# theoneinaminion/FVENS

Measured on AMD Instinct MI355X. Metric: Mfaces/s (flux+residual sweep) + achieved HBM GB/s, 1/2/4/8 MI355X, higher is better.
Workload: dtype f64; 1 GPU; cells=4063232, faces=6359040, boundary_faces=4096, ntheta=2048, nquad=256, ntri=864, farmap=1, parallelism=single GPU

## Files before the change

fvens_amd/csrc/ctx.hpp:

```cpp
#ifndef FVHIP_CTX_HPP
#define FVHIP_CTX_HPP

#include "../../include/fvhip.h"
#include "layout.hpp"
#include "kernels.hpp"
#include "jacobian.hpp"
#include "mesh.hpp"
#include "partition.hpp"
#include "halo.hpp"
#include "ode.hpp"
#include "surface.hpp"
#include "amg.hpp"
#include <rccl/rccl.h>
#include <hip/hip_runtime.h>
#include <cstring>
#include <cstdio>
#include <cstdlib>
#include <algorithm>
#include <cmath>
#include <string>
#include <vector>
#include <map>
#include <stdexcept>
#include <memory>
// ... 91 lines not shown
		double *z = nullptr, *aux = nullptr;
		double *w = nullptr, *t = nullptr, *s = nullptr, *du = nullptr, *yg = nullptr;
		double *jd = nullptr, *jlo = nullptr, *jup = nullptr, *dinv = nullptr;
		float *slo = nullptr, *sup = nullptr, *sdinv = nullptr;
		float* sdiag = nullptr;
		double *part = nullptr, *red = nullptr, *coef = nullptr, *pm = nullptr;
		double *h_red = nullptr, *h_coef = nullptr, *h_red2 = nullptr;
	} iw;
	std::vector<void*> owned_host;
	JacMesh J{};
	bool jac_ready = false;
	double *d_jb = nullptr, *d_jlo = nullptr, *d_jup = nullptr, *d_jdiag = nullptr;
	double* d_raw = nullptr;
	size_t raw_cap = 0;
	double* rawScratch(size_t doubles) {
		if(raw_cap < doubles) {
			if(d_raw) { HC(hipStreamSynchronize(stream)); release(d_raw); }
			d_raw = dalloc(doubles, owned);
			raw_cap = doubles;
		}
		return d_raw;
	}
	int rank = 0, nparts = 1;
	bool rankmesh = false;
	bool use_staged = false;
	bool use_pipe = false;
	int* d_pipe_patch = nullptr;
	hipStream_t stream2 = nullptr;
	std::vector<hipEvent_t> pipe_ev;
	hipEvent_t pipe_start = nullptr, pipe_done = nullptr;
	ncclComm_t comm = nullptr;
	bool in_group = false;
	int* d_fz_order = nullptr;
	hipStream_t comm_stream = nullptr;
	hipEvent_t ev_u = nullptr, ev_halo = nullptr;
	hipEvent_t ev_packed = nullptr, ev_copied = nullptr;
	bool copied_recorded = false;
	int* d_send = nullptr;
	int* d_border = nullptr;
	int nborder = 0;
	double* d_sendbuf = nullptr;
	int* d_trace_conn = nullptr;
	double* d_tracebuf = nullptr;
	int nsend = 0;
	bool prof = false;
	struct Rec { std::string name; hipEvent_t a, b; };
	std::vector<Rec> recs;
	std::map<std::string, std::pair<double,int>> acc;

	~fvhip_ctx() {
		(void)hipSetDevice(device);
		if(comm) (void)ncclCommDestroy(comm);
		for(auto& r : recs) { (void)hipEventDestroy(r.a); (void)hipEventDestroy(r.b); }
		for(hipEvent_t e : pipe_ev) (void)hipEventDestroy(e);
		if(pipe_start) (void)hipEventDestroy(pipe_start);
		if(pipe_done) (void)hipEventDestroy(pipe_done);
		if(stream2) (void)hipStreamDestroy(stream2);
		if(ev_u) (void)hipEventDestroy(ev_u);
		if(ev_halo) (void)hipEventDestroy(ev_halo);
		if(ev_packed) (void)hipEventDestroy(ev_packed);
		if(ev_copied) (void)hipEventDestroy(ev_copied);
		if(comm_stream) (void)hipStreamDestroy(comm_stream);
		for(void* p : owned) (void)hipFree(p);
		for(void* p : owned_host) (void)hipHostFree(p);
		if(stream) (void)hipStreamDestroy(stream);
	}
// ... 89 lines not shown
			HC(hipStreamCreateWithFlags(&stream2, hipStreamNonBlocking));
			pipe_ev.resize(K);
			for(hipEvent_t& e : pipe_ev) HC(hipEventCreateWithFlags(&e, hipEventDisableTiming));
			HC(hipEventCreateWithFlags(&pipe_start, hipEventDisableTiming));
			HC(hipEventCreateWithFlags(&pipe_done, hipEventDisableTiming));
		}
		HC(hipEventRecord(pipe_start, stream));
		HC(hipStreamWaitEvent(stream2, pipe_start, 0));
		for(int k = 0; k < K; k++) {
			timed("k_prep_grad_wls", [&]{
				KOPS(launch_prep_grad_wls)(M, P, u, d_up, d_ubc, d_ug, d_grad, stream, L.pipe_cell_start[k], L.pipe_cell_start[k+1], 0, nullptr);
			});
			HC(hipEventRecord(pipe_ev[k], stream));
		}
		for(int k = 0; k < K; k++) {
			const int n = L.pipe_group_start[k+1] - L.pipe_group_start[k];
			if(n == 0) continue;
			HC(hipStreamWaitEvent(stream2, pipe_ev[k], 0));
			stage_sweep(u, r, dt, dtm, overwrite, d_pipe_patch + L.pipe_group_start[k], n, stream2);
		}
		HC(hipEventRecord(pipe_done, stream2));
		HC(hipStreamWaitEvent(stream, pipe_done, 0));
	}
	void stage_fused(const double* u, double* r, bool dt, double* dtm, bool overwrite,
	                 const int* plist = nullptr, int pcount = 0, hipStream_t st = nullptr) {
		if(!st) st = stream;
		SweepBuffers B{};
		B.u = u; B.r = r; B.dtm = dtm; B.overwrite = overwrite ? 1 : 0;
		B.plist = plist; B.pcount = pcount;
		if(plist && pcount == 0) return;
		B.grad = d_grad;
		if(limited()) B.phi = d_phi;
		B.mfx = mfz.x; B.mfpm = mfz.pm; B.mfres = mfz.res; B.mfmdt = mfz.mdt;
		const char* nm = nullptr;
		timed_on(st, "k_residual_wls", [&]{ nm = KOPS(launch_residual_wls)(M, P, B, cfg.conv_numflux, recKind(), viscKind(),
		                                                                       limKind(), dt, st); });
		if(prof && !recs.empty() && recs.back().name == "k_residual_wls" && nm) recs.back().name = nm;
		HC(hipGetLastError());
	}

	struct MfFuse { const double *x = nullptr, *pm = nullptr, *res = nullptr, *mdt = nullptr; } mfz;
	bool matfreeFusable() const { return fused() && !halo(); }
	bool matfreeNoAlias(const double* u, const double* x, const double* y) const {
		const size_t n = 4*static_cast<size_t>(L.ncell), nt = 4*static_cast<size_t>(L.ncell + L.nghost);
		auto apart = [](const double* a, size_t na, const double* b, size_t nb) { return a + na <= b || b + nb <= a; };
		return apart(y, n, x, nt) && apart(y, n, u, nt);
	}
	void matfree_fused(const double* u, const double* x, const double* pm, const double* res, const double* mdt, double* y) {
		if(!matfreeFusable()) throw std::logic_error("matfree_fused: not a fused single-domain configuration");
		mfz = MfFuse{x, pm, res, mdt};
		try { stage_fused(u, y, false, nullptr, true); }
		catch(...) { mfz = MfFuse{}; throw; }
		mfz = MfFuse{};
	}

	void pack(const double* arr, int width, hipStream_t st = nullptr) {
		if(!st) st = stream;
		timed_on(st, "k_pack", [&]{ launch_pack_rows(d_send, nsend, arr, width, d_sendbuf, st); });
	}
	int sendCount(size_t k, int layers) const {
		return (layers >= 2 || L.send_l1_end.empty() ? L.send_start[k+1] : L.send_l1_end[k]) - L.send_start[k];
	}
	int ghostCount(size_t k, int layers) const {
		return (layers >= 2 || L.ghost_l1_end.empty() ? L.ghost_start[k+1] : L.ghost_l1_end[k]) - L.ghost_start[k];
	}
	void trace_pack(const double* left, int width, hipStream_t st) {
// ... 376 lines not shown
```

fvens_amd/csrc/fvhip_api.cpp:

```cpp
#include "ctx.hpp"

#include <cmath>

namespace fvhip_detail {

fvhip_ctx::GroupExchange groupExchange(const fvhip_group_s* g)
{
	return [g](const fvhip_ctx::ArrayOf& arr_of, int width, int layers) {
		const std::vector<fvhip_ctx*>& hs = g->hs;
		const size_t n = hs.size();
		std::vector<fvhip_ctx*> byrank(n);
		for(fvhip_ctx* h : hs) byrank[h->rank] = h;
		for(size_t i = 0; i < n; i++) if(hs[i]->halo()) { HC(hipSetDevice(hs[i]->device)); hs[i]->pack(arr_of(i), width); }
		for(size_t i = 0; i < n; i++) HC(hipStreamSynchronize(hs[i]->stream));
		for(size_t i = 0; i < n; i++) {
			fvhip_ctx* h = hs[i];
			const Layout& L = h->L;
			for(size_t k = 0; k < L.nbr_rank.size(); k++) {
				fvhip_ctx* q = byrank[L.nbr_rank[k]];
				const Layout& Q = q->L;
				size_t kk = 0;
				while(kk < Q.nbr_rank.size() && Q.nbr_rank[kk] != h->rank) kk++;
				if(kk == Q.nbr_rank.size()) throw std::logic_error("halo lists are not symmetric");
				const int cnt = h->ghostCount(k, layers);
// ... 57 lines not shown
	DevMesh& M = h->M;
	M.ncell = L.ncell + L.nghost; M.nown = L.ncell; M.nbface = L.nbface;
	M.npatch = static_cast<int>(L.patch_cell.size()) - 1;
	M.nslot = static_cast<int>(L.slot_L.size());
	M.patch_cell = upload(L.patch_cell, o);
	M.patch_slot = upload(L.patch_slot, o);
	M.slot_LR = reinterpret_cast<const int2*>(upload(pack2(L.slot_L, L.slot_R), o));
	M.slot_n = reinterpret_cast<const double2*>(upload(L.slot_n, o));
	M.slot_len = upload(L.slot_len, o);
	M.slot_gr = reinterpret_cast<const double2*>(upload(L.slot_gr, o));
	M.cell_slots = reinterpret_cast<const int4*>(upload(L.cell_slots, o));
	M.cell_nbr = reinterpret_cast<const int4*>(upload(L.cell_nbr_local, o));
	M.cell_face = reinterpret_cast<const int4*>(upload(L.cell_face_local, o));
	M.cell_nbr_fo = reinterpret_cast<const int4*>(upload(L.cell_nbr_fo, o));
	M.rc = reinterpret_cast<const double2*>(upload(L.rc, o));
	M.area = upload(L.area, o);
	M.wls_V = reinterpret_cast<const double4*>(upload(L.wls_V, o));
	M.venk_eps2 = upload(L.venk_eps2, o);
	M.bf_L = upload(L.bf_L, o);
	M.bf_bc = upload(L.bf_bc, o);
	M.bf_n = reinterpret_cast<const double2*>(upload(L.bf_n, o));
	M.bf_rcbp = reinterpret_cast<const double2*>(upload(L.bf_rcbp, o));
	if(!L.fz_ext_start.empty()) {
		M.fz_ext_start = upload(L.fz_ext_start, o);
		M.fz_ext = upload(L.fz_ext, o);
		M.fz_n1 = upload(L.fz_n1, o);
		M.fz_g_start = upload(L.fz_g_start, o);
		M.fz_gnbr = reinterpret_cast<const int4*>(upload(L.fz_gnbr, o));
		M.fz_slot_lr16 = upload(L.fz_slot_lr16, o);
		M.fz_gnbr16 = reinterpret_cast<const uint2*>(upload(L.fz_gnbr16, o));
		M.fz_gbf_start = upload(L.fz_gbf_start, o);
		M.fz_gbf = upload(L.fz_gbf, o);
		M.fz_cslot16 = reinterpret_cast<const uint2*>(upload(L.fz_cslot16, o));
		M.fz_max_cells = L.fz_max_cells;
	}
	M.gg_n = static_cast<int>(L.gg_cells.size());
	M.gg_cells = upload(L.gg_cells, o);
	M.gg_nbr = reinterpret_cast<const int4*>(upload(L.gg_nbr, o));
	M.gg_V = reinterpret_cast<const double4*>(upload(L.gg_V, o));
	M.gg_gp = reinterpret_cast<const double2*>(upload(L.gg_gp, o));
	M.gg_eps2 = upload(L.gg_eps2, o);
	M.xb_bc = upload(L.xb_bc, o);
	M.xb_n = reinterpret_cast<const double2*>(upload(L.xb_n, o));
	M.xb_rcbp = reinterpret_cast<const double2*>(upload(L.xb_rcbp, o));
	if(!L.pipe_patch.empty()) h->d_pipe_patch = upload(L.pipe_patch, o);
	if(L.nghost > 0 && !L.fz_order.empty()) h->d_fz_order = upload(L.fz_order, o);
	h->d_perm = upload(L.perm, o);
	h->nsend = static_cast<int>(L.send_cells.size());
	h->nborder = static_cast<int>(L.border_cells.size());
	if(h->nborder > 0) h->d_border = upload(L.border_cells, o);
	if(h->nsend > 0) {
		h->d_send = upload(L.send_cells, o);
		h->d_sendbuf = dalloc(8*static_cast<size_t>(h->nsend), o);
	}
	if(!L.trace_conn.empty()) {
		if(static_cast<int>(L.trace_conn.size()) != h->nsend) throw std::logic_error("per-rank mesh: trace lists differ");
		h->d_trace_conn = upload(L.trace_conn, o);
		h->d_tracebuf = dalloc(4*static_cast<size_t>(L.nghost), o);
	}

	DevPhys& P = h->P;
	P.gas = gd::make_gas(cfg->gamma, cfg->Minf, cfg->Tinf, cfg->Reinf, cfg->Pr);
	const double beta = 0;
	P.uinf[0] = 1.0;
	P.uinf[1] = std::cos(cfg->aoa)*std::cos(beta);
	P.uinf[2] = std::sin(cfg->aoa)*std::cos(beta);
// ... 634 lines not shown
			names[static_cast<size_t>(n)*namelen + namelen-1] = '\0';
			ms[n] = kv.second.first; counts[n] = kv.second.second;
			n++;
		}
	});
	return rc ? -1 : n;
}

static void layoutStats(const Layout& L, long long* s, int n)
{
	long long v[16] = {};
	v[0] = L.ncell; v[1] = L.naface; v[2] = static_cast<long long>(L.slot_L.size());
	v[3] = static_cast<long long>(L.patch_cell.size()) - 1; v[4] = L.max_slots; v[5] = L.nbface;
	v[6] = L.nghost; v[7] = static_cast<long long>(L.nbr_rank.size()); v[8] = static_cast<long long>(L.send_cells.size());
	v[9] = L.fz_ninner;
	v[10] = static_cast<long long>(L.fz_ext.size()) - L.fz_ring2;
	const long long np = static_cast<long long>(L.patch_cell.size()) - 1;
	if(!L.fz_ext_start.empty())
		for(long long p = 0; p < np; p++) {
			const long long nl = (L.patch_cell[p+1] - L.patch_cell[p]) + (L.fz_ext_start[p+1] - L.fz_ext_start[p]);
			if(nl > SLOTS_MAX) v[11]++;
		}
	v[12] = L.fz_ring2;
	v[13] = L.fz_max_cells;
	v[14] = SLOTS_MAX;
	for(int i = 0; i < n && i < 16; i++) s[i] = v[i];
}

int fvhip_layout_stats(fvhip_handle h, long long* s)
{
	return guard([&] { need(h, "handle"); need(s, "stats"); layoutStats(h->L, s, 12); });
}

int fvhip_layout_probe(const fvhip_mesh* mesh, const fvhip_flow_config* cfg, long long* s)
{
	return guard([&] {
		if(!mesh || !cfg || !s) throw std::invalid_argument("null argument");
		checkConfig(cfg);
		const Layout L = buildLayout(topoFromMesh(*mesh), *cfg, true);
		layoutStats(L, s, 16);
	});
}

int fvhip_local_flux(int flux_type, const double* gas5, int nf, const double* ul, const double* ur,
                     const double* n, double* flux)
{
	return guard([&] {
		const gd::Gas G = gd::make_gas(gas5[0], gas5[1], gas5[2], gas5[3], gas5[4]);
		double *a, *b, *c, *d;
		HC(hipMalloc(&a, 4*sizeof(double)*nf + 8)); HC(hipMalloc(&b, 4*sizeof(double)*nf + 8));
		HC(hipMalloc(&c, 2*sizeof(double)*nf + 8)); HC(hipMalloc(&d, 4*sizeof(double)*nf + 8));
		HC(hipMemcpy(a, ul, 4*sizeof(double)*nf, hipMemcpyHostToDevice));
		HC(hipMemcpy(b, ur, 4*sizeof(double)*nf, hipMemcpyHostToDevice));
		HC(hipMemcpy(c, n, 2*sizeof(double)*nf, hipMemcpyHostToDevice));
		exact::launch_local_flux(flux_type, G, nf, a, b, c, d, nullptr);
		HC(hipGetLastError());
		HC(hipMemcpy(flux, d, 4*sizeof(double)*nf, hipMemcpyDeviceToHost));
		(void)hipFree(a); (void)hipFree(b); (void)hipFree(c); (void)hipFree(d);
	});
}

int fvhip_divsqrt_probe(int n, const double* a, const double* b, double* out)
{
	return guard([&] {
		double *da, *db, *dout;
		HC(hipMalloc(&da, sizeof(double)*n + 8)); HC(hipMalloc(&db, sizeof(double)*n + 8));
// ... 157 lines not shown
```

fvens_amd/csrc/kernels.hip:

```cpp
#include "kernels.hpp"
#include "layout.hpp"
#include <algorithm>
#include <mutex>
#include <set>
#include <stdexcept>
#include <string>

#ifndef FVHIP_NS
#define FVHIP_NS exact
#endif

namespace fvhip {
namespace FVHIP_NS {

using namespace gd;

__device__ __forceinline__ int xcd_chunk(int nchunk) {
	const int q = (nchunk + 7) >> 3;
	return (static_cast<int>(blockIdx.x) & 7) * q + (static_cast<int>(blockIdx.x) >> 3);
}
static inline int xcd_blocks(long long nchunk) { return static_cast<int>(8*((nchunk + 7)/8)); }

__device__ __forceinline__ void ld4(const double* p, int i, double* o) {
	const double4 v = reinterpret_cast<const double4*>(p)[i];
// ... 985 lines not shown
		grad[1][3] = davg[1] - ddr*dr[1] + corr*dr[1];
	}
	#pragma unroll
	for(int i = 1; i < 3; i++) {
		__asm__ volatile("" ::: "memory");
		const double tl = rowi[i], tr = rowj ? rowj[i] : (i == 1 ? gpr.y : gpr.z);
		double davg[2];
		davg[0] = 0.5*(rowi[4 + i*2 + 0] + gsrc[4 + i*2 + 0]);
		davg[1] = 0.5*(rowi[4 + i*2 + 1] + gsrc[4 + i*2 + 1]);
		const double corr = div_rn(tr-tl, dist);
		const double ddr = dot2(davg,dr);
		grad[0][i] = davg[0] - ddr*dr[0] + corr*dr[0];
		grad[1][i] = davg[1] - ddr*dr[1] + corr*dr[1];
	}
	const double kd = div_rcp(muRe, G.kden, G.rkden);
	double ldiv = 0;
	ldiv += grad[0][1]; ldiv += grad[1][2];
	ldiv *= 2.0/3.0*muRe;
	double s[2][2];
	s[0][0] = __builtin_fma(muRe*grad[0][1], 2.0, -ldiv); s[0][1] = muRe*(grad[0][2] + grad[1][1]);
	s[1][0] = muRe*(grad[1][1] + grad[0][2]); s[1][1] = __builtin_fma(muRe*grad[1][2], 2.0, -ldiv);
	vf[0] = 0;
	for(int i = 0; i < 2; i++) { double t = 0; t -= s[i][0]*n[0]; t -= s[i][1]*n[1]; vf[i+1] = t; }
	double e = 0;
	for(int i = 0; i < 2; i++) {
		double comp = 0;
		comp += s[i][0]*va[0]; comp += s[i][1]*va[1];
		comp += kd*grad[i][3];
		e -= comp * n[i];
	}
	vf[3] = e;
}

struct FzPatch { int p, s0, s1, c0, c1, nc, e0, nl, ng; const uint2* gnbr; const int* gbf; };
struct FzPre { int cf; double ua[4]; double2 rca; int4 nb4a; int2 lrl; double2 nn; double len;
               double2 gpa[4]; double eps2a; };

__device__ __forceinline__ FzPatch fz_patch(const DevMesh& M, const SweepBuffers& B, int pi)
{
	FzPatch q;
	q.p = B.plist ? B.plist[pi] : pi;
	q.s0 = M.patch_slot[q.p]; q.s1 = M.patch_slot[q.p+1];
	q.c0 = M.patch_cell[q.p]; q.c1 = M.patch_cell[q.p+1];
	q.nc = q.c1 - q.c0;
	q.e0 = M.fz_ext_start[q.p];
	q.nl = q.nc + (M.fz_ext_start[q.p+1] - q.e0);
	q.ng = q.nc + M.fz_n1[q.p];
	q.gnbr = M.fz_gnbr16 + M.fz_g_start[q.p];
	q.gbf = M.fz_gbf + M.fz_gbf_start[q.p];
	return q;
}
__device__ __forceinline__ int fz_nbr_code(unsigned x, const int* gbf)
{
	if(x == 0xFFFFu) return -1;
	if(x & 0x8000u) return -2 - gbf[x & 0x7FFFu];
	return static_cast<int>(x);
}
__device__ __forceinline__ int4 fz_nbrs(const FzPatch& q, int i)
{
	const uint2 v = q.gnbr[i];
	return make_int4(fz_nbr_code(v.x & 0xFFFFu, q.gbf), fz_nbr_code(v.x >> 16, q.gbf),
	                 fz_nbr_code(v.y & 0xFFFFu, q.gbf), fz_nbr_code(v.y >> 16, q.gbf));
}
__device__ __forceinline__ int fz_cell(const DevMesh& M, const FzPatch& q, int i)
{
	return i < q.nc ? q.c0 + i : M.fz_ext[q.e0 + (i - q.nc)];
}
template <bool MF>
__device__ __forceinline__ void fz_load_rows(const DevMesh& M, const SweepBuffers& B, const FzPatch& q, int t, FzPre& a)
{
	a.ua[0] = a.ua[1] = a.ua[2] = a.ua[3] = 0.0;
	a.rca = make_double2(0, 0);
	if(t < q.nl) { ld_state<MF>(B, a.cf, a.ua); a.rca = M.rc[a.cf]; }
	const int s = q.s0 + t;
	a.lrl = make_int2(0, -1); a.nn = make_double2(0, 0); a.len = 0;
	if(s < q.s1) {
		const unsigned v = M.fz_slot_lr16[s];
		a.lrl = make_int2(static_cast<int>(v & 0xFFFFu), (v >> 16) == 0xFFFFu ? -2 : static_cast<int>(v >> 16));
		a.nn = M.slot_n[s]; a.len = M.slot_len[s];
	}
}
__device__ __forceinline__ void fz_load_grad(const DevMesh& M, const FzPatch& q, int t, FzPre& a)
{
	a.nb4a = make_int4(-1, -1, -1, -1);
	if(t < q.ng && a.cf < M.nown) a.nb4a = fz_nbrs(q, t);
}

template <int FLUX, int REC, bool DT, int VISC, int LIM, typename HA, typename HB>
__device__ __forceinline__ void fz_body(const DevMesh& M, const DevPhys& P, const SweepBuffers& B, double* fz,
                                        const FzPatch& q, const FzPre& a, HA&& hookA, HB&& hookB)
{
	const Gas& G = P.gas;
	const int t = static_cast<int>(threadIdx.x);
	const int s = q.s0 + t;
	constexpr int W = fz_w<VISC>();

	if(t < q.nl) stage_row(G, &fz[t*W], a.ua, a.rca);
	for(int i = t + SLOTS_MAX; i < q.nl; i += SLOTS_MAX) {
		const int c = fz_cell(M, q, i);
		double b[4];
		ld_state<!DT>(B, c, b);
		stage_row(G, &fz[i*W], b, M.rc[c]);
	}
	__syncthreads();

	hookA();
	if(t < q.ng) fused_wls_row<LIM, W, !DT>(M, P, B, fz, &fz[t*W], a.cf, a.nb4a, LIM ? a.gpa : nullptr, a.eps2a);
	for(int i = t + SLOTS_MAX; i < q.ng; i += SLOTS_MAX) {
		const int c = fz_cell(M, q, i);
		fused_wls_row<LIM, W, !DT>(M, P, B, fz, &fz[i*W], c, c < M.nown ? fz_nbrs(q, i) : make_int4(-1, -1, -1, -1));
	}
	__syncthreads();

	double f[4] = {0, 0, 0, 0};
	double sri = 0, srj = 0;
	if(s < q.s1) {
		const int2 lrl = a.lrl;
		const double2 nn = a.nn;
		const double flen = a.len;
		const double n[2] = {nn.x, nn.y};
		const bool bnd = lrl.y < -1;
		int bf = 0, bcell = 0;
		if(bnd) { const int2 g = M.slot_LR[s]; bf = g.y - M.ncell; bcell = g.x; }
		double ul[4], ur[4];
		const double* rowi = &fz[lrl.x*W];
		const double2 ri = *reinterpret_cast<const double2*>(rowi + 12);
		double ui[4], gi[8];
		ld4(rowi, 0, ui);
		ld8(rowi + 4, 0, gi);
		if(REC == SR_MUSCL) {
			if(!bnd) {
				const double* rowj = &fz[lrl.y*W];
				const double2 rj = *reinterpret_cast<const double2*>(rowj + 12);
				double uj[4], gj[8];
				ld4(rowj, 0, uj);
				ld8(rowj + 4, 0, gj);
				const double dx = rj.x-ri.x, dy = rj.y-ri.y;
				#pragma unroll
				for(int i = 0; i < 4; i++) {
					double dl = mul0(gi[i*2], dx); dl += gi[i*2+1]*dy;
					double dr = mul0(gj[i*2], dx); dr += gj[i*2+1]*dy;
					const double du = uj[i] - ui[i];
					const double dm = twice_minus(dl, du);
					const double dp = twice_minus(dr, du);
					ul[i] = muscl_left(ui[i], uj[i], dm, muscl_phi(dm, du));
// ... 62 lines not shown
				if(g.x < M.nown) sri += div_rn(div_rcp(coi*mui, G.Pr, G.rPr) * flen*flen, M.area[g.x]);
				if(!bnd && g.y < M.nown) srj += div_rn(div_rcp(coj*muj, G.Pr, G.rPr) * flen*flen, M.area[g.y]);
			}
		}
		if(VISC != SV_NONE) {
			double muRe, va[2];
			viscous_face_terms_mu<VISC == SV_CONST>(G, ul, ur, mui, muj, muRe, va);
			double4 gpr = make_double4(0, 0, 0, 0);
			const double* rowj = nullptr;
			double2 rr;
			if(bnd) { gpr = ghost_prim_of_cell<!DT>(M, P, B, bcell, bf); rr = M.bf_rcbp[bf]; }
			else { rowj = &fz[lrl.y*W]; rr = *reinterpret_cast<const double2*>(rowj + 12); }
			const double4 vg = make_double4(ri.x, ri.y, rr.x, rr.y);
			double vf[4] = {0, 0, 0, 0};
			fz_viscous(G, rowi, rowj, gpr, vg, n, muRe, va, vf);
			#pragma unroll
			for(int k = 0; k < 4; k++) f[k] += vf[k]*flen;
		}
	}
	hookB();
	const int c = q.c0 + t;
	uint2 cs = make_uint2(0xFFFFFFFFu, 0xFFFFFFFFu);
	double carea = 0.0;
	if(c < q.c1) { cs = M.fz_cslot16[c]; if(DT) carea = M.area[c]; }
	__syncthreads();
	double* sf = fz;
	double* ssr = fz + 4*SLOTS_MAX;
	if(s < q.s1) {
		sf[0*SLOTS_MAX + t] = f[0]; sf[1*SLOTS_MAX + t] = f[1];
		sf[2*SLOTS_MAX + t] = f[2]; sf[3*SLOTS_MAX + t] = f[3];
		if(DT) { ssr[t] = sri; ssr[SLOTS_MAX + t] = srj; }
	}
	__syncthreads();

	if(c < q.c1) {
		double r[4];
		if(B.overwrite) { r[0] = r[1] = r[2] = r[3] = 0.0; }
		else ld4(B.r, c, r);
		double integ = 0.0;
		const unsigned e[4] = {cs.x & 0xFFFFu, cs.x >> 16, cs.y & 0xFFFFu, cs.y >> 16};
		#pragma unroll
		for(int k = 0; k < 4; k++) {
			if(e[k] == 0xFFFFu) break;
			const int ls = static_cast<int>(e[k] >> 1);
			if(e[k] & 1) {
				r[0] += sf[0*SLOTS_MAX + ls]; r[1] += sf[1*SLOTS_MAX + ls];
				r[2] += sf[2*SLOTS_MAX + ls]; r[3] += sf[3*SLOTS_MAX + ls];
				if(DT) integ += ssr[SLOTS_MAX + ls];
			} else {
				r[0] -= sf[0*SLOTS_MAX + ls]; r[1] -= sf[1*SLOTS_MAX + ls];
				r[2] -= sf[2*SLOTS_MAX + ls]; r[3] -= sf[3*SLOTS_MAX + ls];
				if(DT) integ += ssr[ls];
			}
		}
		if(!DT && B.mfx) {
			double x[4], rs[4];
			ld4(B.mfx, c, x);
			ld4(B.mfres, c, rs);
			const double d = B.mfmdt[c], pert = B.mfpm[1];
			#pragma unroll
			for(int i = 0; i < 4; i++) r[i] = d*x[i] + (-r[i] + rs[i])/pert;
		}
		st4(B.r, c, r);
		if(DT) B.dtm[c] = div_rn(carea, integ);
	}
}

#ifndef FVHIP_FUSED_WAVES
#define FVHIP_FUSED_WAVES 5
#endif
#ifndef FVHIP_FUSED_WAVES_LIM
#define FVHIP_FUSED_WAVES_LIM 4
#endif
#ifndef FVHIP_FUSED_WAVES_VISC
#define FVHIP_FUSED_WAVES_VISC 4
#endif

template <int FLUX, int REC, bool DT, int VISC, int LIM>
__global__ void __launch_bounds__(SLOTS_MAX, VISC != SV_NONE ? FVHIP_FUSED_WAVES_VISC : (LIM ? FVHIP_FUSED_WAVES_LIM : FVHIP_FUSED_WAVES)) k_residual_wls(const DevMesh M, const DevPhys P, const SweepBuffers B)
{
	extern __shared__ __attribute__((aligned(16))) double fz[];
	const int np = B.plist ? B.pcount : M.npatch;
	const int t = static_cast<int>(threadIdx.x);
	const int q = (np + 7) >> 3;
	const int pi = (blockIdx.x & 7) * q + (blockIdx.x >> 3);
	if(pi >= np) return;
	const FzPatch cur = fz_patch(M, B, pi);
	FzPre pre;
	pre.cf = t < cur.nl ? fz_cell(M, cur, t) : 0;
	fz_load_rows<!DT>(M, B, cur, t, pre);
	fz_load_grad(M, cur, t, pre);
	pre.eps2a = 0.0;
	if(LIM) {
		const bool own = t < cur.ng && pre.cf < M.nown;
		fz_face_centres(M, own ? pre.cf : 0, pre.gpa);
		if(LIM == 2) pre.eps2a = M.venk_eps2[own ? pre.cf : 0];
	}
	fz_body<FLUX, REC, DT, VISC, LIM>(M, P, B, fz, cur, pre, []() {}, []() {});
}

__global__ void k_fill(double* p, double v, long long n)
{
	const long long i = static_cast<long long>(blockIdx.x)*blockDim.x + threadIdx.x;
	if(i < n) p[i] = v;
}

__global__ void k_local_flux(int type, Gas G, int nf, const double* ul, const double* ur, const double* n, double* f)
{
	const int i = blockIdx.x*blockDim.x + threadIdx.x;
	if(i >= nf) return;
	double a[4], b[4], o[4];
	ld4(ul, i, a); ld4(ur, i, b);
	const double nn[2] = {n[2*i], n[2*i+1]};
	inviscid_flux_rt(type, G, a, b, nn, o);
	st4(f, i, o);
}

__global__ void k_gather(const int* perm, const double* src, double* dst, int n, int width)
{
	const long long i = static_cast<long long>(blockIdx.x)*blockDim.x + threadIdx.x;
	if(i >= static_cast<long long>(n)*width) return;
	const int c = static_cast<int>(i / width), w = static_cast<int>(i % width);
	dst[i] = src[static_cast<size_t>(perm[c])*width + w];
}

__global__ void k_scatter(const int* perm, const double* src, double* dst, int n, int width)
{
	const long long i = static_cast<long long>(blockIdx.x)*blockDim.x + threadIdx.x;
	if(i >= static_cast<long long>(n)*width) return;
	const int c = static_cast<int>(i / width), w = static_cast<int>(i % width);
	dst[static_cast<size_t>(perm[c])*width + w] = src[i];
// ... 150 lines not shown
const char* launch_residual_wls(const DevMesh& M, const DevPhys& P, const SweepBuffers& B, int flux, int rec,
                                int visc, int lim, bool dt, hipStream_t s)
{
	FusedFn fn;
	switch(flux) {
		case 0: fn = pickFused<0>(rec, visc, lim, dt); break;
		case 1: fn = pickFused<1>(rec, visc, lim, dt); break;
		case 2: fn = pickFused<2>(rec, visc, lim, dt); break;
		case 3: fn = pickFused<3>(rec, visc, lim, dt); break;
		case 4: fn = pickFused<4>(rec, visc, lim, dt); break;
		case 5: fn = pickFused<5>(rec, visc, lim, dt); break;
		default: fn = pickFused<6>(rec, visc, lim, dt); break;
	}
	const size_t W = visc != SV_NONE ? FZW_VISC : FZW;
	const size_t lds = std::max(static_cast<size_t>(M.fz_max_cells)*W, static_cast<size_t>(6*SLOTS_MAX))*sizeof(double);
	{
		static std::mutex mu;
		static std::set<std::pair<const void*, int>> configured;
		int dev = 0;
		if(hipGetDevice(&dev) != hipSuccess) throw std::runtime_error("k_residual_wls: hipGetDevice failed");
		std::lock_guard<std::mutex> lock(mu);
		if(configured.insert({reinterpret_cast<const void*>(fn), dev}).second) {
			const size_t maxlds = std::max(static_cast<size_t>(FUSED_LDS_CELLS)*W, static_cast<size_t>(6*SLOTS_MAX))*sizeof(double);
			const hipError_t e = hipFuncSetAttribute(reinterpret_cast<const void*>(fn),
			                                         hipFuncAttributeMaxDynamicSharedMemorySize, static_cast<int>(maxlds));
			if(e != hipSuccess) {
				configured.erase({reinterpret_cast<const void*>(fn), dev});
				throw std::runtime_error(std::string("k_residual_wls: raising the dynamic LDS limit failed: ")
				                         + hipGetErrorString(e));
			}
		}
	}
	const int np = B.plist ? B.pcount : M.npatch;
	if(np > 0) hipLaunchKernelGGL(fn, dim3(8*((np + 7)/8)), dim3(SLOTS_MAX), lds, s, M, P, B);
	return kFusedNames[flux < 0 || flux > 6 ? 6 : flux];
}

}
}
```

fvens_amd/csrc/kernels.hpp:

```cpp
#ifndef FVHIP_KERNELS_HPP
#define FVHIP_KERNELS_HPP

#include <hip/hip_runtime.h>
#include "gasdyn.hpp"

namespace fvhip {

constexpr int MAXBC = 16;

enum SweepRec { SR_FIRST = 0, SR_MUSCL = 1, SR_LINEAR = 2 };
enum SweepVisc { SV_NONE = 0, SV_SUTHERLAND = 1, SV_CONST = 2 };

struct DevMesh
{
	int ncell;
	int nown;
	int nbface, npatch, nslot;
	const int* patch_cell;
	const int* patch_slot;
	const int2* slot_LR;
	const double2* slot_n;
	const double* slot_len;
	const double2* slot_gr;
	const int4* cell_slots;
	const int4* cell_nbr;
	const int4* cell_face;
	const int4* cell_nbr_fo;
	const double2* rc;
	const double* area;
	const double4* wls_V;
	const double* venk_eps2;
	const int* bf_L;
	const int* bf_bc;
	const double2* bf_n;
	const double2* bf_rcbp;
	const int* fz_ext_start;
	const int* fz_ext;
	const int* fz_n1;
	const int* fz_g_start;
	const int4* fz_gnbr;
	const unsigned* fz_slot_lr16;
	const uint2* fz_gnbr16;
	const int* fz_gbf_start;
	const int* fz_gbf;
	const uint2* fz_cslot16;
	int fz_max_cells;
	int gg_n;
	const int* gg_cells;
	const int4* gg_nbr;
	const double4* gg_V;
	const double2* gg_gp;
	const double* gg_eps2;
	const int* xb_bc;
	const double2* xb_n;
	const double2* xb_rcbp;
};

struct DevPhys
{
	gd::Gas gas;
	double uinf[4];
	gd::BCDev bc[MAXBC];
	int nbc;
	double limiter_param;
};

struct SweepBuffers
{
	const double* u;
	const double* up;
	const double* grad;
	const double* rgrad;
	const double* phi;
	const double* ubc;
	const double* ug;
	double* r;
	double* dtm;
	int overwrite;
	const int* plist;
	int pcount;
	const double* mfx;
	const double* mfpm;
	const double* mfres;
	const double* mfmdt;
};

#define FVHIP_SWEEP_LAUNCHERS \
void launch_prep(const DevMesh& M, const DevPhys& P, const double* u, double* up, double* ubc, double* ug, \
                 bool cells, hipStream_t s); \
void launch_grad_wls(const DevMesh& M, const double* up, const double* ug, double* grad, hipStream_t s); \
void launch_prep_grad_wls(const DevMesh& M, const DevPhys& P, const double* u, double* up, double* ubc, \
                          double* ug, double* grad, hipStream_t s, int c_begin = 0, int c_end = -1, \
                          int lim = 0, double* phi = nullptr); \
void launch_grad_wls_list(const DevMesh& M, const DevPhys& P, const double* u, const int* list, int n, \
                          double* grad, hipStream_t s); \
void launch_grad_ghost(const DevMesh& M, const DevPhys& P, const double* u, double* grad, hipStream_t s, \
                       int lim = 0, double* phi = nullptr); \
void launch_grad_gg(const DevMesh& M, const double* up, const double* ug, double* grad, hipStream_t s); \
void launch_limiter(const DevMesh& M, const DevPhys& P, int venk, const double* up, const double* ug, \
                    const double* grad, double* phi, hipStream_t s); \
void launch_weno(const DevMesh& M, const DevPhys& P, const double* grad, double* lgrad, hipStream_t s); \
 \
const char* launch_sweep(const DevMesh& M, const DevPhys& P, const SweepBuffers& B, int flux, int rec, \
                         int visc, bool dt, hipStream_t s); \
const char* launch_residual_wls(const DevMesh& M, const DevPhys& P, const SweepBuffers& B, int flux, int rec, \
                                int visc, int lim, bool dt, hipStream_t s); \
void launch_fill(double* p, double v, long long n, hipStream_t s); \
void launch_local_flux(int flux, const gd::Gas& G, int nf, const double* ul, const double* ur, \
                       const double* n, double* f, hipStream_t s); \
void launch_gather_cells(const int* perm, const double* src, double* dst, int n, int width, hipStream_t s); \
void launch_scatter_cells(const int* perm, const double* src, double* dst, int n, int width, hipStream_t s); \
void launch_divsqrt_probe(int n, const double* a, const double* b, double* out, hipStream_t s);

namespace exact { FVHIP_SWEEP_LAUNCHERS }
namespace fast { FVHIP_SWEEP_LAUNCHERS }

}
// ... 2 lines not shown
```

fvens_amd/csrc/layout.cpp:

```cpp
#include <cstdlib>
#include "layout.hpp"
#include "partition.hpp"
#include <algorithm>
#include <numeric>
#include <stdexcept>
#include <string>
#include <cmath>

namespace fvhip {

namespace {

inline uint64_t hilbertD(uint32_t n, uint32_t x, uint32_t y)
{
	uint64_t d = 0;
	for(uint32_t s = n/2; s > 0; s /= 2) {
		const uint32_t rx = (x & s) > 0, ry = (y & s) > 0;
		d += static_cast<uint64_t>(s) * s * ((3 * rx) ^ ry);
		if(ry == 0) {
			if(rx == 1) { x = s-1 - x; y = s-1 - y; }
			const uint32_t t = x; x = y; y = t;
		}
	}
	return d;
// ... 493 lines not shown
			Lo.fz_slot_lr[2*static_cast<size_t>(s)] = code(Lo.slot_L[s]);
			Lo.fz_slot_lr[2*static_cast<size_t>(s)+1] = code(Lo.slot_R[s]);
		}
		const size_t gb0 = Lo.fz_gbf.size();
		for(size_t k = Lo.fz_gnbr.size() - 4*static_cast<size_t>(ng); k < Lo.fz_gnbr.size(); k++) {
			const int v = Lo.fz_gnbr[k];
			if(v == -1) { Lo.fz_gnbr16.push_back(0xFFFF); continue; }
			if(v >= 0) { Lo.fz_gnbr16.push_back(static_cast<uint16_t>(v)); continue; }
			const size_t j = Lo.fz_gbf.size() - gb0;
			if(j >= 0x7FFF) throw std::logic_error("fused residual: too many boundary faces in one patch");
			Lo.fz_gbf.push_back(-2 - v);
			Lo.fz_gnbr16.push_back(static_cast<uint16_t>(0x8000 | j));
		}
		Lo.fz_gbf_start.push_back(static_cast<int>(Lo.fz_gbf.size()));
		for(int s = Lo.patch_slot[p]; s < Lo.patch_slot[p+1]; s++) {
			const int l = Lo.fz_slot_lr[2*static_cast<size_t>(s)], r = Lo.fz_slot_lr[2*static_cast<size_t>(s)+1];
			Lo.fz_slot_lr16[s] = static_cast<uint32_t>(l) | (static_cast<uint32_t>(r >= 0 ? r : 0xFFFF) << 16);
		}
		for(int c = c0; c < c1; c++)
			for(int j = 0; j < MAXF; j++) {
				const int e = Lo.cell_slots[static_cast<size_t>(c)*MAXF+j];
				if(e < 0) continue;
				const int ls = (e >> 1) - Lo.patch_slot[p];
				if(ls < 0 || ls >= SLOTS_MAX) throw std::logic_error("fused residual: cell face outside its patch");
				Lo.fz_cslot16[static_cast<size_t>(c)*MAXF+j] = static_cast<uint16_t>((ls << 1) | (e & 1));
			}
		Lo.fz_max_cells = std::max(Lo.fz_max_cells, nl);
		bool inner = true;
		for(size_t k = e0; k < Lo.fz_ext.size(); k++) if(Lo.fz_ext[k] >= Lo.ncell) inner = false;
		innerp[p] = inner ? 1 : 0;
		for(int c = c0; c < c1; c++) lidx[c] = -1;
		for(size_t k = e0; k < Lo.fz_ext.size(); k++) lidx[Lo.fz_ext[k]] = -1;
	}
	Lo.fz_order.clear();
	for(int p = 0; p < npatch; p++) if(innerp[p]) Lo.fz_order.push_back(p);
	Lo.fz_ninner = static_cast<int>(Lo.fz_order.size());
	for(int p = 0; p < npatch; p++) if(!innerp[p]) Lo.fz_order.push_back(p);
}

}
```

fvens_amd/csrc/layout.hpp:

```cpp
#ifndef FVHIP_LAYOUT_HPP
#define FVHIP_LAYOUT_HPP

#include <vector>
#include <cstdint>
#include "../../include/fvhip.h"

namespace fvhip {

#ifndef FVHIP_SLOTS
#define FVHIP_SLOTS 256
#endif
#ifndef FVHIP_FUSED_ROWS
#define FVHIP_FUSED_ROWS (FVHIP_SLOTS*11/8)
#endif
constexpr int SLOTS_MAX = FVHIP_SLOTS;
constexpr int CELLS_MAX = FVHIP_SLOTS;
constexpr int MAXF = 4;

struct Layout
{
	int ncell = 0;
	int nghost = 0;
	int nbface = 0, naface = 0, ninface = 0;
	std::vector<int> perm;
	std::vector<int> iperm;
	std::vector<int> patch_cell;
	std::vector<int> patch_slot;
	std::vector<int> slot_L, slot_R;
	std::vector<int> slot_face;
	std::vector<double> slot_n;
	std::vector<double> slot_len;
	std::vector<double> slot_gr;
	std::vector<int> cell_slots;
	std::vector<int> cell_nbr_local;
	std::vector<int> cell_face_local;
	std::vector<int> cell_nbr_fo;
	std::vector<int> cell_nfael;
	std::vector<double> rc;
	std::vector<double> area;
	std::vector<double> wls_V;
// ... 4 lines not shown
	std::vector<double> bf_rcbp;
	std::vector<int> bf_tag;
	std::vector<double> bf_gr;
	std::vector<int> if_L, if_R;
	std::vector<int> if_slot;
	std::vector<double> if_n, if_len;
	std::vector<double> bf_len;
	std::vector<int> cell_rfaces;
	int max_slots = 0;
	std::vector<int> nbr_rank, ghost_start, send_start, send_cells;
	std::vector<int> border_cells;
	int halo_layers = 1;
	std::vector<int> ghost_l1_end, send_l1_end;
	std::vector<int> gg_cells;
	std::vector<int> gg_nbr;
	std::vector<double> gg_V;
	std::vector<double> gg_gp;
	std::vector<double> gg_eps2;
	std::vector<int> xb_bc;
	std::vector<double> xb_n, xb_rcbp;
	std::vector<int> cell_global;
	std::vector<int> trace_conn;
	std::vector<int> fz_ext_start;
	std::vector<int> fz_ext;
	std::vector<int> fz_n1;
	std::vector<int> fz_g_start;
	std::vector<int> fz_gnbr;
	std::vector<int> fz_slot_lr;
	std::vector<uint32_t> fz_slot_lr16;
	std::vector<uint16_t> fz_gnbr16;
	std::vector<int> fz_gbf_start;
	std::vector<int> fz_gbf;
	std::vector<uint16_t> fz_cslot16;
	int fz_ring2 = 0;
	int fz_max_cells = 0;
	int fz_row_cap = 0;
	std::vector<int> fz_order;
	int fz_ninner = 0;
	std::vector<int> pipe_cell_start;
	std::vector<int> pipe_patch;
	std::vector<int> pipe_group_start;
};

constexpr int FUSED_LDS_CELLS = FVHIP_FUSED_ROWS;
constexpr int FUSED_LDS_CELLS_5W = FVHIP_SLOTS*284/256;
int fusedRowCap(const fvhip_flow_config& cfg);
static_assert(FUSED_LDS_CELLS < 0x8000 && 2*SLOTS_MAX < 0xFFFF, "fused codes are 16-bit");
constexpr int PIPE_CHUNKS = 8;

bool fusedEligible(const fvhip_flow_config& cfg);
void buildFused(Layout& Lo);

bool pipelineEligible(const fvhip_flow_config& cfg);
void buildPipeline(Layout& Lo, int chunks);

Layout buildLayout(const fvhip_mesh& m, const fvhip_flow_config& cfg, bool renumber);
struct MeshTopo;
Layout buildLayout(const MeshTopo& T, const fvhip_flow_config& cfg, bool renumber);

}
#endif
```

Measured before the change: 26180 Mfaces/s.

## Pack per-patch metadata into one 32-byte record and hoist all first-phase loads

Replaces the roughly ten scattered per-patch index loads (patch_slot, patch_cell, fz_ext_start, fz_n1, fz_g_start, fz_gbf_start) with a single aligned 32-byte record unpacked in registers. It also merges the row, gradient-stencil and limiter face-centre loads into one function that issues every independent global load up front, so their latencies overlap before the first barrier. The aim is to shorten the dependent-load chain at kernel entry. The cost is more live registers during that phase, which could lower occupancy. Optional timestamp instrumentation behind a compile flag and host-side consistency checks are added too.

```diff
diff --git a/fvens_amd/csrc/ctx.hpp b/fvens_amd/csrc/ctx.hpp
--- a/fvens_amd/csrc/ctx.hpp
+++ b/fvens_amd/csrc/ctx.hpp
@@ -147,6 +147,10 @@
 	ncclComm_t comm = nullptr;
 	bool in_group = false;
 	int* d_fz_order = nullptr;
+#ifdef FVHIP_FZ_STAMPS
+	unsigned long long* d_stamps = nullptr;
+	long long stamp_blocks = 0;
+#endif
 	hipStream_t comm_stream = nullptr;
 	hipEvent_t ev_u = nullptr, ev_halo = nullptr;
 	hipEvent_t ev_packed = nullptr, ev_copied = nullptr;
@@ -302,6 +306,20 @@
 		B.grad = d_grad;
 		if(limited()) B.phi = d_phi;
 		B.mfx = mfz.x; B.mfpm = mfz.pm; B.mfres = mfz.res; B.mfmdt = mfz.mdt;
+#ifdef FVHIP_FZ_STAMPS
+		{
+			const size_t words = 8*static_cast<size_t>(8*((M.npatch + 7)/8));
+			if(!d_stamps) {
+				void* p = nullptr;
+				HC(hipMalloc(&p, words*sizeof(unsigned long long)));
+				owned.push_back(p);
+				d_stamps = static_cast<unsigned long long*>(p);
+			}
+			HC(hipMemsetAsync(d_stamps, 0, words*sizeof(unsigned long long), st));
+			B.stamps = d_stamps;
+			stamp_blocks = 8*(((plist ? pcount : M.npatch) + 7)/8);
+		}
+#endif
 		const char* nm = nullptr;
 		timed_on(st, "k_residual_wls", [&]{ nm = KOPS(launch_residual_wls)(M, P, B, cfg.conv_numflux, recKind(), viscKind(),
 		                                                                       limKind(), dt, st); });
diff --git a/fvens_amd/csrc/fvhip_api.cpp b/fvens_amd/csrc/fvhip_api.cpp
--- a/fvens_amd/csrc/fvhip_api.cpp
+++ b/fvens_amd/csrc/fvhip_api.cpp
@@ -113,6 +113,7 @@
 		M.fz_gbf_start = upload(L.fz_gbf_start, o);
 		M.fz_gbf = upload(L.fz_gbf, o);
 		M.fz_cslot16 = reinterpret_cast<const uint2*>(upload(L.fz_cslot16, o));
+		M.fz_rec = upload(L.fz_rec, o);
 		M.fz_max_cells = L.fz_max_cells;
 	}
 	M.gg_n = static_cast<int>(L.gg_cells.size());
@@ -813,6 +814,22 @@
 	return guard([&] { need(h, "handle"); need(s, "stats"); layoutStats(h->L, s, 12); });
 }
 
+#ifdef FVHIP_FZ_STAMPS
+int fvhip_debug_fz_stamps(fvhip_ctx* h, unsigned long long* out, long long cap, long long* nblocks, int* wall_khz)
+{
+	return guard([&] {
+		if(!h || !out || !nblocks || !wall_khz) throw std::invalid_argument("null argument");
+		if(!h->d_stamps) throw std::logic_error("no fused residual has run on this handle");
+		HC(hipSetDevice(h->device));
+		HC(hipStreamSynchronize(h->stream));
+		if(cap < 8*h->stamp_blocks) throw std::invalid_argument("stamp buffer too small");
+		HC(hipMemcpy(out, h->d_stamps, 8*static_cast<size_t>(h->stamp_blocks)*sizeof(unsigned long long), hipMemcpyDeviceToHost));
+		*nblocks = h->stamp_blocks;
+		HC(hipDeviceGetAttribute(wall_khz, hipDeviceAttributeWallClockRate, h->device));
+	});
+}
+#endif
+
 int fvhip_layout_probe(const fvhip_mesh* mesh, const fvhip_flow_config* cfg, long long* s)
 {
 	return guard([&] {
diff --git a/fvens_amd/csrc/kernels.hip b/fvens_amd/csrc/kernels.hip
--- a/fvens_amd/csrc/kernels.hip
+++ b/fvens_amd/csrc/kernels.hip
@@ -1041,6 +1041,23 @@
 	vf[3] = e;
 }
 
+#ifdef FVHIP_FZ_STAMPS
+struct FzStamps { unsigned long long t[7], w0; };
+#define FZ_STAMPS_PARAM , FzStamps& stamps
+#define FZ_STAMPS_ARG , stamps
+#define FZ_STAMP(k) do { asm volatile("" ::: "memory"); stamps.t[k] = __builtin_amdgcn_s_memtime(); \
+                         asm volatile("" ::: "memory"); } while(0)
+#define FZ_STAMP_ENTRY() asm("s_memtime %0\n\ts_waitcnt lgkmcnt(0)" : "=s"(stamps.t[0]) : "s"(blockIdx.x))
+#define FZ_STAMP_AFTER(k, a, b, c, d) asm("s_memtime %0\n\ts_waitcnt lgkmcnt(0)" : "=s"(stamps.t[k]) \
+                                          : "s"(a), "s"(b), "s"(c), "s"(d))
+#else
+#define FZ_STAMPS_PARAM
+#define FZ_STAMPS_ARG
+#define FZ_STAMP(k) do {} while(0)
+#define FZ_STAMP_ENTRY() do {} while(0)
+#define FZ_STAMP_AFTER(k, a, b, c, d) do {} while(0)
+#endif
+
 struct FzPatch { int p, s0, s1, c0, c1, nc, e0, nl, ng; const uint2* gnbr; const int* gbf; };
 struct FzPre { int cf; double ua[4]; double2 rca; int4 nb4a; int2 lrl; double2 nn; double len;
                double2 gpa[4]; double eps2a; };
@@ -1049,14 +1066,15 @@
 {
 	FzPatch q;
 	q.p = B.plist ? B.plist[pi] : pi;
-	q.s0 = M.patch_slot[q.p]; q.s1 = M.patch_slot[q.p+1];
-	q.c0 = M.patch_cell[q.p]; q.c1 = M.patch_cell[q.p+1];
-	q.nc = q.c1 - q.c0;
-	q.e0 = M.fz_ext_start[q.p];
-	q.nl = q.nc + (M.fz_ext_start[q.p+1] - q.e0);
-	q.ng = q.nc + M.fz_n1[q.p];
-	q.gnbr = M.fz_gnbr16 + M.fz_g_start[q.p];
-	q.gbf = M.fz_gbf + M.fz_gbf_start[q.p];
+	const FzPatchMeta m = fz_unpack(M.fz_rec[q.p]);
+	q.s0 = m.s0; q.s1 = m.s0 + m.ns;
+	q.c0 = m.c0; q.c1 = m.c0 + m.nc;
+	q.nc = m.nc;
+	q.e0 = m.e0;
+	q.nl = m.nl;
+	q.ng = m.ng;
+	q.gnbr = M.fz_gnbr16 + m.g0;
+	q.gbf = M.fz_gbf + m.gbf0;
 	return q;
 }
 __device__ __forceinline__ int fz_nbr_code(unsigned x, const int* gbf)
@@ -1065,39 +1083,64 @@
 	if(x & 0x8000u) return -2 - gbf[x & 0x7FFFu];
 	return static_cast<int>(x);
 }
-__device__ __forceinline__ int4 fz_nbrs(const FzPatch& q, int i)
-{
-	const uint2 v = q.gnbr[i];
-	return make_int4(fz_nbr_code(v.x & 0xFFFFu, q.gbf), fz_nbr_code(v.x >> 16, q.gbf),
-	                 fz_nbr_code(v.y & 0xFFFFu, q.gbf), fz_nbr_code(v.y >> 16, q.gbf));
-}
+__device__ __forceinline__ int4 fz_nbr_codes(uint2 v, const int* gbf)
+{
+	return make_int4(fz_nbr_code(v.x & 0xFFFFu, gbf), fz_nbr_code(v.x >> 16, gbf),
+	                 fz_nbr_code(v.y & 0xFFFFu, gbf), fz_nbr_code(v.y >> 16, gbf));
+}
+__device__ __forceinline__ int4 fz_nbrs(const FzPatch& q, int i) { return fz_nbr_codes(q.gnbr[i], q.gbf); }
 __device__ __forceinline__ int fz_cell(const DevMesh& M, const FzPatch& q, int i)
 {
 	return i < q.nc ? q.c0 + i : M.fz_ext[q.e0 + (i - q.nc)];
 }
-template <bool MF>
-__device__ __forceinline__ void fz_load_rows(const DevMesh& M, const SweepBuffers& B, const FzPatch& q, int t, FzPre& a)
-{
-	a.ua[0] = a.ua[1] = a.ua[2] = a.ua[3] = 0.0;
-	a.rca = make_double2(0, 0);
-	if(t < q.nl) { ld_state<MF>(B, a.cf, a.ua); a.rca = M.rc[a.cf]; }
+template <bool MF, int LIM>
+__device__ __forceinline__ void fz_load_first(const DevMesh& M, const SweepBuffers& B, const FzPatch& q, int t, FzPre& a)
+{
+	const bool own = t < q.nc, ring = !own && t < q.nl, grow = t < q.ng;
+	int cr = 0;
+	if(ring) cr = M.fz_ext[q.e0 + (t - q.nc)];
+	const int co = q.c0 + (own ? t : 0);
+	double uo[4];
+	ld_state<MF>(B, co, uo);
+	const double2 rco = M.rc[co];
 	const int s = q.s0 + t;
+	const bool face = s < q.s1;
+	const int sc = face ? s : q.s0;
+	const unsigned v = M.fz_slot_lr16[sc];
+	const double2 nn = M.slot_n[sc];
+	const double len = M.slot_len[sc];
+	const uint2 codes = q.gnbr[grow ? t : 0];
+	int4 cs = make_int4(-1, -1, -1, -1);
+	if(LIM) cs = M.cell_slots[co];
+	a.cf = own ? co : cr;
+	#pragma unroll
+	for(int k = 0; k < 4; k++) a.ua[k] = uo[k];
+	a.rca = rco;
+	if(ring) {
+		ld_state<MF>(B, cr, a.ua);
+		a.rca = M.rc[cr];
+		if(LIM && grow && cr < M.nown) cs = M.cell_slots[cr];
+	}
 	a.lrl = make_int2(0, -1); a.nn = make_double2(0, 0); a.len = 0;
-	if(s < q.s1) {
-		const unsigned v = M.fz_slot_lr16[s];
+	if(face) {
 		a.lrl = make_int2(static_cast<int>(v & 0xFFFFu), (v >> 16) == 0xFFFFu ? -2 : static_cast<int>(v >> 16));
-		a.nn = M.slot_n[s]; a.len = M.slot_len[s];
-	}
-}
-__device__ __forceinline__ void fz_load_grad(const DevMesh& M, const FzPatch& q, int t, FzPre& a)
-{
+		a.nn = nn; a.len = len;
+	}
 	a.nb4a = make_int4(-1, -1, -1, -1);
-	if(t < q.ng && a.cf < M.nown) a.nb4a = fz_nbrs(q, t);
+	if(grow) a.nb4a = fz_nbr_codes(codes, q.gbf);
+	a.eps2a = 0.0;
+	if(LIM) {
+		const bool og = grow && a.cf < M.nown;
+		const int sl[4] = {cs.x, cs.y, cs.z, cs.w};
+		#pragma unroll
+		for(int k = 0; k < 4; k++) a.gpa[k] = sl[k] >= 0 ? M.slot_gr[sl[k] >> 1] : make_double2(0, 0);
+		if(LIM == 2) a.eps2a = M.venk_eps2[og ? a.cf : 0];
+	}
 }
 
 template <int FLUX, int REC, bool DT, int VISC, int LIM, typename HA, typename HB>
 __device__ __forceinline__ void fz_body(const DevMesh& M, const DevPhys& P, const SweepBuffers& B, double* fz,
-                                        const FzPatch& q, const FzPre& a, HA&& hookA, HB&& hookB)
+                                        const FzPatch& q, const FzPre& a, HA&& hookA, HB&& hookB FZ_STAMPS_PARAM)
 {
 	const Gas& G = P.gas;
 	const int t = static_cast<int>(threadIdx.x);
@@ -1111,7 +1154,9 @@
 		ld_state<!DT>(B, c, b);
 		stage_row(G, &fz[i*W], b, M.rc[c]);
 	}
+	FZ_STAMP(2);
 	__syncthreads();
+	FZ_STAMP(3);
 
 	hookA();
 	if(t < q.ng) fused_wls_row<LIM, W, !DT>(M, P, B, fz, &fz[t*W], a.cf, a.nb4a, LIM ? a.gpa : nullptr, a.eps2a);
@@ -1120,6 +1165,7 @@
 		fused_wls_row<LIM, W, !DT>(M, P, B, fz, &fz[i*W], c, c < M.nown ? fz_nbrs(q, i) : make_int4(-1, -1, -1, -1));
 	}
 	__syncthreads();
+	FZ_STAMP(4);
 
 	double f[4] = {0, 0, 0, 0};
 	double sri = 0, srj = 0;
@@ -1248,6 +1294,7 @@
 		if(DT) { ssr[t] = sri; ssr[SLOTS_MAX + t] = srj; }
 	}
 	__syncthreads();
+	FZ_STAMP(5);
 
 	if(c < q.c1) {
 		double r[4];
@@ -1280,6 +1327,7 @@
 		st4(B.r, c, r);
 		if(DT) B.dtm[c] = div_rn(carea, integ);
 	}
+	FZ_STAMP(6);
 }
 
 #ifndef FVHIP_FUSED_WAVES
@@ -1296,23 +1344,28 @@
 __global__ void __launch_bounds__(SLOTS_MAX, VISC != SV_NONE ? FVHIP_FUSED_WAVES_VISC : (LIM ? FVHIP_FUSED_WAVES_LIM : FVHIP_FUSED_WAVES)) k_residual_wls(const DevMesh M, const DevPhys P, const SweepBuffers B)
 {
 	extern __shared__ __attribute__((aligned(16))) double fz[];
+#ifdef FVHIP_FZ_STAMPS
+	FzStamps stamps;
+	asm("s_memrealtime %0\n\ts_waitcnt lgkmcnt(0)" : "=s"(stamps.w0) : "s"(blockIdx.y));
+#endif
+	FZ_STAMP_ENTRY();
 	const int np = B.plist ? B.pcount : M.npatch;
 	const int t = static_cast<int>(threadIdx.x);
 	const int q = (np + 7) >> 3;
 	const int pi = (blockIdx.x & 7) * q + (blockIdx.x >> 3);
 	if(pi >= np) return;
 	const FzPatch cur = fz_patch(M, B, pi);
+	FZ_STAMP_AFTER(1, cur.s1, cur.nl, cur.ng, cur.c0);
 	FzPre pre;
-	pre.cf = t < cur.nl ? fz_cell(M, cur, t) : 0;
-	fz_load_rows<!DT>(M, B, cur, t, pre);
-	fz_load_grad(M, cur, t, pre);
-	pre.eps2a = 0.0;
-	if(LIM) {
-		const bool own = t < cur.ng && pre.cf < M.nown;
-		fz_face_centres(M, own ? pre.cf : 0, pre.gpa);
-		if(LIM == 2) pre.eps2a = M.venk_eps2[own ? pre.cf : 0];
-	}
-	fz_body<FLUX, REC, DT, VISC, LIM>(M, P, B, fz, cur, pre, []() {}, []() {});
+	fz_load_first<!DT, LIM>(M, B, cur, t, pre);
+	fz_body<FLUX, REC, DT, VISC, LIM>(M, P, B, fz, cur, pre, []() {}, []() {} FZ_STAMPS_ARG);
+#ifdef FVHIP_FZ_STAMPS
+	if(t == 0 && B.stamps) {
+		unsigned long long* o = B.stamps + 8*static_cast<size_t>(blockIdx.x);
+		for(int k = 0; k < 7; k++) o[k] = stamps.t[k];
+		o[7] = wall_clock64() - stamps.w0;
+	}
+#endif
 }
 
 __global__ void k_fill(double* p, double v, long long n)
@@ -1529,7 +1582,7 @@
 		}
 	}
 	const int np = B.plist ? B.pcount : M.npatch;
-	if(np > 0) hipLaunchKernelGGL(fn, dim3(8*((np + 7)/8)), dim3(SLOTS_MAX), lds, s, M, P, B);
+	if(np > 0 && M.nown > 0) hipLaunchKernelGGL(fn, dim3(8*((np + 7)/8)), dim3(SLOTS_MAX), lds, s, M, P, B);
 	return kFusedNames[flux < 0 || flux > 6 ? 6 : flux];
 }
 
diff --git a/fvens_amd/csrc/kernels.hpp b/fvens_amd/csrc/kernels.hpp
--- a/fvens_amd/csrc/kernels.hpp
+++ b/fvens_amd/csrc/kernels.hpp
@@ -3,6 +3,7 @@
 
 #include <hip/hip_runtime.h>
 #include "gasdyn.hpp"
+#include "layout.hpp"
 
 namespace fvhip {
 
@@ -44,6 +45,7 @@
 	const int* fz_gbf_start;
 	const int* fz_gbf;
 	const uint2* fz_cslot16;
+	const FzPatchRec* fz_rec;
 	int fz_max_cells;
 	int gg_n;
 	const int* gg_cells;
@@ -83,6 +85,9 @@
 	const double* mfpm;
 	const double* mfres;
 	const double* mfmdt;
+#ifdef FVHIP_FZ_STAMPS
+	unsigned long long* stamps;
+#endif
 };
 
 #define FVHIP_SWEEP_LAUNCHERS \
diff --git a/fvens_amd/csrc/layout.cpp b/fvens_amd/csrc/layout.cpp
--- a/fvens_amd/csrc/layout.cpp
+++ b/fvens_amd/csrc/layout.cpp
@@ -549,6 +549,35 @@
 		for(int c = c0; c < c1; c++) lidx[c] = -1;
 		for(size_t k = e0; k < Lo.fz_ext.size(); k++) lidx[Lo.fz_ext[k]] = -1;
 	}
+	Lo.fz_rec.assign(npatch, FzPatchRec{});
+	for(int p = 0; p < npatch; p++) {
+		const int nc = Lo.patch_cell[p+1] - Lo.patch_cell[p], ns = Lo.patch_slot[p+1] - Lo.patch_slot[p];
+		const int n1 = Lo.fz_n1[p], nx = Lo.fz_ext_start[p+1] - Lo.fz_ext_start[p];
+		for(int v : {nc, ns, n1, nx})
+			if(v < 0 || v > 0xFFFF) throw std::logic_error("fused residual: a patch count does not fit in 16 bits");
+		if(Lo.ncell > 0 && (nc < 1 || ns < 1)) throw std::logic_error("fused residual: patch without a cell or a face");
+		FzPatchRec& r = Lo.fz_rec[p];
+		r.s0 = Lo.patch_slot[p]; r.c0 = Lo.patch_cell[p]; r.e0 = Lo.fz_ext_start[p];
+		r.g0 = Lo.fz_g_start[p]; r.gbf0 = Lo.fz_gbf_start[p];
+		r.nc_ns = static_cast<uint32_t>(nc) | (static_cast<uint32_t>(ns) << 16);
+		r.n1_nx = static_cast<uint32_t>(n1) | (static_cast<uint32_t>(nx) << 16);
+		r.spare = 0;
+	}
+	for(int p = 0; p < npatch; p++) {
+		const FzPatchMeta m = fz_unpack(Lo.fz_rec[p]);
+		const bool same = m.s0 == Lo.patch_slot[p] && m.s0 + m.ns == Lo.patch_slot[p+1]
+			&& m.c0 == Lo.patch_cell[p] && m.c0 + m.nc == Lo.patch_cell[p+1]
+			&& m.e0 == Lo.fz_ext_start[p] && m.e0 + (m.nl - m.nc) == Lo.fz_ext_start[p+1]
+			&& m.ng == m.nc + Lo.fz_n1[p] && m.g0 == Lo.fz_g_start[p] && m.g0 + m.ng == Lo.fz_g_start[p+1]
+			&& m.gbf0 == Lo.fz_gbf_start[p];
+		if(!same) throw std::logic_error("fused residual: patch record differs from the arrays it packs");
+		for(int i = m.nc; i < m.ng; i++) {
+			if(Lo.fz_ext[m.e0 + (i - m.nc)] < Lo.ncell) continue;
+			const uint16_t* g = &Lo.fz_gnbr16[4*static_cast<size_t>(m.g0 + i)];
+			if(g[0] != 0xFFFF || g[1] != 0xFFFF || g[2] != 0xFFFF || g[3] != 0xFFFF)
+				throw std::logic_error("fused residual: a ghost gradient row has neighbour codes");
+		}
+	}
 	Lo.fz_order.clear();
 	for(int p = 0; p < npatch; p++) if(innerp[p]) Lo.fz_order.push_back(p);
 	Lo.fz_ninner = static_cast<int>(Lo.fz_order.size());
diff --git a/fvens_amd/csrc/layout.hpp b/fvens_amd/csrc/layout.hpp
--- a/fvens_amd/csrc/layout.hpp
+++ b/fvens_amd/csrc/layout.hpp
@@ -4,8 +4,28 @@
 #include <vector>
 #include <cstdint>
 #include "../../include/fvhip.h"
+#include "gasdyn.hpp"
 
 namespace fvhip {
+
+struct alignas(32) FzPatchRec
+{
+	int32_t s0, c0, e0, g0, gbf0;
+	uint32_t nc_ns;
+	uint32_t n1_nx;
+	uint32_t spare;
+};
+static_assert(sizeof(FzPatchRec) == 32, "FzPatchRec is eight 32-bit words");
+struct FzPatchMeta { int s0, ns, c0, nc, e0, nl, ng, g0, gbf0; };
+FVHIP_HD FzPatchMeta fz_unpack(const FzPatchRec& r)
+{
+	FzPatchMeta m;
+	m.s0 = r.s0; m.c0 = r.c0; m.e0 = r.e0; m.g0 = r.g0; m.gbf0 = r.gbf0;
+	m.nc = static_cast<int>(r.nc_ns & 0xFFFFu); m.ns = static_cast<int>(r.nc_ns >> 16);
+	m.ng = m.nc + static_cast<int>(r.n1_nx & 0xFFFFu);
+	m.nl = m.nc + static_cast<int>(r.n1_nx >> 16);
+	return m;
+}
 
 #ifndef FVHIP_SLOTS
 #define FVHIP_SLOTS 256
@@ -76,6 +96,7 @@
 	std::vector<int> fz_gbf_start;
 	std::vector<int> fz_gbf;
 	std::vector<uint16_t> fz_cslot16;
+	std::vector<FzPatchRec> fz_rec;
 	int fz_ring2 = 0;
 	int fz_max_cells = 0;
 	int fz_row_cap = 0;
```

After: 26740 Mfaces/s, median of 6. 1.02x the previous value.
